# lucidrains/audiolm-pytorch

Hardware: NVIDIA H100
Metric: CoarseTransformer tokens/sec fwd+bwd seq2048 (higher is better)
Workload: dtype bf16

## Files before the change

audiolm_pytorch_b200/csrc/attn_fwd_wgmma.cu:

```cuda
#include "alm_common.cuh"
#include "ptx_sm90.cuh"

namespace alm {

constexpr int ATT_BM = 128;
constexpr int ATT_BN = 128;
constexpr int ATT_THREADS = 384;
template <int D>
struct AttFwdCfg {
  static constexpr int KV_STAGES = D == 128 ? 3 : 4;
  static constexpr int HALF_BYTES = 128 * SwizzledTile<D>::ROW_BYTES;
  static constexpr int TILE_BYTES = 128 * D * 2;
  static constexpr int SMEM_BYTES = TILE_BYTES * (1 + 2 * KV_STAGES) + 256;
};

struct AttnFwdParams {
  __nv_bfloat16* o;
  float* lse;
  const uint32_t* kmask;
  int kb_stride;
  const float* bias;
  long long bias_hs, bias_rs;
  long long ldo, lse_stride;
  int b, h, n_q, n_k;
  int causal;
  float scale_log2;
  int n_q_pad;
  uint32_t drop_row0;
  DropoutArgs drop;
};

__device__ __forceinline__ float att_ex2(float x) {
  float y;
  asm("ex2.approx.ftz.f32 %0, %1;" : "=f"(y) : "f"(x));
  return y;
}

__device__ __forceinline__ uint64_t attn_fwd_keep_bits(const DropoutArgs& d, uint32_t qrow, uint32_t kbase, int c_lane) {
  const uint32_t odd = qrow & 1u;
  uint64_t bits = 0;
#pragma unroll
  for (int kk = 0; kk < ATT_BN / 16; ++kk) {
    const uint32_t j0 = kbase + 16 * kk + c_lane;
    const uint4 own = dropout_draw(d, qrow, j0 + odd);
    const uint32_t ra = __shfl_xor_sync(0xffffffffu, odd ? own.x : own.y, 4);
    const uint32_t rb = __shfl_xor_sync(0xffffffffu, odd ? own.z : own.w, 4);
    const uint4 other = odd ? make_uint4(0u, ra, 0u, rb) : make_uint4(ra, 0u, rb, 0u);
#pragma unroll
    for (int c = 0; c < 2; ++c) {
      const uint4 dr = (uint32_t)c == odd ? own : other;
#pragma unroll
      for (int half = 0; half < 2; ++half)
#pragma unroll
        for (int h = 0; h < 2; ++h)
          if (dropout_pick(d, dr, qrow + 8 * h, j0 + 8 * half + c)) bits |= 1ull << (8 * kk + 4 * half + 2 * h + c);
    }
  }
  return bits;
}

template <int ATT_D, bool HAS_BIAS, bool DROPOUT>
__global__ void __launch_bounds__(ATT_THREADS, 1)
mqa_attn_fwd_kernel(const __grid_constant__ CUtensorMap tmQ, const __grid_constant__ CUtensorMap tmK,
                    const __grid_constant__ CUtensorMap tmV, const AttnFwdParams p) {
  using Tile = SwizzledTile<ATT_D>;
  using Cfg = AttFwdCfg<ATT_D>;
  constexpr int ATT_KV_STAGES = Cfg::KV_STAGES, ATT_TILE_BYTES = Cfg::TILE_BYTES, HALF = Cfg::HALF_BYTES;
  constexpr bool REG_HANDOFF = ATT_D == 128;
  extern __shared__ __align__(1024) uint8_t smem_raw[];
  uint8_t* smem = smem_raw;
  if ((smem_u32(smem) & 1023u) != 0) __trap();
  uint8_t* sQ = smem;
  uint8_t* sK = sQ + ATT_TILE_BYTES;
  uint8_t* sV = sK + ATT_KV_STAGES * ATT_TILE_BYTES;
  uint64_t* bars = reinterpret_cast<uint64_t*>(sV + ATT_KV_STAGES * ATT_TILE_BYTES);
  uint64_t* q_full = bars;
  uint64_t* kv_full = bars + 1;
  uint64_t* kv_empty = kv_full + ATT_KV_STAGES;

  const int warp = threadIdx.x >> 5;
  const int lane = threadIdx.x & 31;
  const int wg = warp >> 2;
  const int n_qblocks = (p.n_q + ATT_BM - 1) / ATT_BM;
  const int qb = n_qblocks - 1 - (int)blockIdx.x;
  const int head = blockIdx.y;
  const int batch = blockIdx.z;
  const int q0 = qb * ATT_BM;
  const int off = p.n_k - p.n_q;
  int kv_end = p.n_k;
  if (p.causal) kv_end = min(p.n_k, q0 + ATT_BM + off);
  const int n_tiles = kv_end > 0 ? (kv_end + ATT_BN - 1) / ATT_BN : 0;

  if (threadIdx.x == 0) {
    tma_prefetch_desc(&tmQ);
    tma_prefetch_desc(&tmK);
    tma_prefetch_desc(&tmV);
    mbar_init(q_full, 1);
    for (int i = 0; i < ATT_KV_STAGES; ++i) {
      mbar_init(&kv_full[i], 1);
      mbar_init(&kv_empty[i], 8);
    }
    fence_mbar_init();
  }
  __syncthreads();

  if (wg == 0) {
    if constexpr (REG_HANDOFF) setmaxnreg_dec<40>();
    if (warp == 0 && n_tiles > 0) {
      if (elect_one_sync()) {
        mbar_arrive_expect_tx(q_full, ATT_TILE_BYTES);
#pragma unroll
        for (int hf = 0; hf < Tile::HALVES; ++hf)
          tma_load_3d(sQ + hf * HALF, &tmQ, q_full, head * ATT_D + hf * Tile::HW, q0, batch);
      }
      __syncwarp();
      int stage = 0;
      uint32_t phase = 0;
      for (int j = 0; j < n_tiles; ++j) {
        mbar_wait(&kv_empty[stage], phase ^ 1u);
        if (elect_one_sync()) {
          mbar_arrive_expect_tx(&kv_full[stage], 2 * ATT_TILE_BYTES);
#pragma unroll
          for (int hf = 0; hf < Tile::HALVES; ++hf) {
            tma_load_3d(sK + stage * ATT_TILE_BYTES + hf * HALF, &tmK, &kv_full[stage], hf * Tile::HW, j * ATT_BN, batch);
            tma_load_3d(sV + stage * ATT_TILE_BYTES + hf * HALF, &tmV, &kv_full[stage], hf * Tile::HW, j * ATT_BN, batch);
          }
        }
        __syncwarp();
        if (++stage == ATT_KV_STAGES) { stage = 0; phase ^= 1u; }
      }
    }
    return;
  }

  if constexpr (REG_HANDOFF) setmaxnreg_inc<232>();
  const int cw = wg - 1;
  const int r_base = cw * 64 + (warp & 3) * 16 + (lane >> 2);
  const int c_lane = 2 * (lane & 3);
  constexpr float kLog2e = 1.4426950408889634f;
  float m_run[2] = {-INFINITY, -INFINITY}, l_run[2] = {0.f, 0.f};
  float o_acc[ATT_D / 2];
#pragma unroll
  for (int d = 0; d < ATT_D / 2; ++d) o_acc[d] = 0.f;
  int q_limit[2];
  [[maybe_unused]] const float* brow[2];
#pragma unroll
  for (int h = 0; h < 2; ++h) {
    const int qi = q0 + r_base + 8 * h;
    q_limit[h] = min(p.causal ? qi + off : p.n_k - 1, p.n_k - 1);
    if constexpr (HAS_BIAS) brow[h] = p.bias + (long long)head * p.bias_hs + (long long)min(qi, p.n_q - 1) * p.bias_rs;
  }
  const uint32_t* mrow = p.kmask ? p.kmask + (long long)batch * p.kb_stride : nullptr;
  const uint32_t q_addr = smem_u32(sQ) + cw * 64 * Tile::ROW_BYTES;
  [[maybe_unused]] const uint32_t drop_row =
      p.drop_row0 + ((uint32_t)batch * p.h + head) * (uint32_t)p.n_q_pad + q0 + r_base;

  if (n_tiles > 0) mbar_wait(q_full, 0);
  int stage = 0;
  uint32_t phase = 0;
  for (int j = 0; j < n_tiles; ++j) {
    mbar_wait(&kv_full[stage], phase);
    const uint32_t k_addr = smem_u32(sK + stage * ATT_TILE_BYTES);
    const uint32_t v_addr = smem_u32(sV + stage * ATT_TILE_BYTES);
    float s[ATT_BN / 2];
    wgmma_fence();
#pragma unroll
    for (int k = 0; k < ATT_D / 16; ++k)
      wgmma_ss<ATT_BN>(s, Tile::kmajor(q_addr, k, HALF), Tile::kmajor(k_addr, k, HALF), k > 0 ? 1u : 0u);
    wgmma_commit();
    [[maybe_unused]] uint64_t keep = 0;
    if constexpr (DROPOUT) keep = attn_fwd_keep_bits(p.drop, drop_row, j * ATT_BN, c_lane);
    wgmma_wait<0>();
    wgmma_fence_acc(s);

    const int kbase = j * ATT_BN;
    const bool tile_full = mrow == nullptr && kbase + ATT_BN <= p.n_k && (!p.causal || kbase + ATT_BN - 1 <= q0 + off);
    uint32_t valid[4] = {0xFFFFFFFFu, 0xFFFFFFFFu, 0xFFFFFFFFu, 0xFFFFFFFFu};
    if (!tile_full && mrow != nullptr) {
      const uint4 mv = __ldg(reinterpret_cast<const uint4*>(mrow + j * 4));
      valid[0] = mv.x; valid[1] = mv.y; valid[2] = mv.z; valid[3] = mv.w;
    }
    uint32_t pa[ATT_BN / 16][4];
#pragma unroll
    for (int h = 0; h < 2; ++h) {
#pragma unroll
      for (int g = 0; g < ATT_BN / 8; ++g)
#pragma unroll
        for (int c = 0; c < 2; ++c) {
          const int col = 8 * g + c_lane + c;
          float v = s[4 * g + 2 * h + c] * p.scale_log2;
          if constexpr (HAS_BIAS) {
            if (kbase + col < p.bias_rs) v = fmaf(__ldg(brow[h] + kbase + col), kLog2e, v);
          }
          if (!tile_full) {
            const bool ok = kbase + col <= q_limit[h] && ((valid[col >> 5] >> (col & 31)) & 1u);
            if (!ok) v = -INFINITY;
          }
          s[4 * g + 2 * h + c] = v;
        }
      float m_tile = -INFINITY;
#pragma unroll
      for (int g = 0; g < ATT_BN / 8; ++g) m_tile = fmaxf(m_tile, fmaxf(s[4 * g + 2 * h], s[4 * g + 2 * h + 1]));
      m_tile = fmaxf(m_tile, __shfl_xor_sync(0xffffffffu, m_tile, 1));
      m_tile = fmaxf(m_tile, __shfl_xor_sync(0xffffffffu, m_tile, 2));
      const float m_new = fmaxf(m_run[h], m_tile);
      const float m_use = (m_new == -INFINITY) ? 0.f : m_new;
      const float alpha = att_ex2(m_run[h] - m_use);
      float l_tile = 0.f;
#pragma unroll
      for (int g = 0; g < ATT_BN / 8; ++g)
#pragma unroll
        for (int c = 0; c < 2; ++c) {
          const float pv = att_ex2(s[4 * g + 2 * h + c] - m_use);
          s[4 * g + 2 * h + c] = pv;
          l_tile += pv;
        }
      l_run[h] = fmaf(l_run[h], alpha, l_tile);
      m_run[h] = m_new;
#pragma unroll
      for (int g = 0; g < ATT_D / 8; ++g) {
        o_acc[4 * g + 2 * h] *= alpha;
        o_acc[4 * g + 2 * h + 1] *= alpha;
      }
    }
    if constexpr (DROPOUT) {
#pragma unroll
      for (int e = 0; e < ATT_BN / 2; ++e) s[e] = ((keep >> e) & 1u) ? s[e] * p.drop.scale : 0.f;
    }
#pragma unroll
    for (int kk = 0; kk < ATT_BN / 16; ++kk) {
      pa[kk][0] = pack_bf16x2(s[8 * kk + 0], s[8 * kk + 1]);
      pa[kk][1] = pack_bf16x2(s[8 * kk + 2], s[8 * kk + 3]);
      pa[kk][2] = pack_bf16x2(s[8 * kk + 4], s[8 * kk + 5]);
      pa[kk][3] = pack_bf16x2(s[8 * kk + 6], s[8 * kk + 7]);
    }
    wgmma_fence_acc(o_acc);
    wgmma_fence();
#pragma unroll
    for (int kk = 0; kk < ATT_BN / 16; ++kk)
      wgmma_rs<ATT_D, 1>(o_acc, pa[kk], Tile::mnmajor(v_addr, kk, HALF), 1u);
    wgmma_commit();
    wgmma_wait<0>();
    wgmma_fence_acc(o_acc);
    if (lane == 0) mbar_arrive(&kv_empty[stage]);
    if (++stage == ATT_KV_STAGES) { stage = 0; phase ^= 1u; }
  }

#pragma unroll
  for (int h = 0; h < 2; ++h) {
    float l_tot = l_run[h];
    l_tot += __shfl_xor_sync(0xffffffffu, l_tot, 1);
    l_tot += __shfl_xor_sync(0xffffffffu, l_tot, 2);
    const int qi = q0 + r_base + 8 * h;
    if (qi < p.n_q) {
      const float inv = l_tot > 0.f ? 1.f / l_tot : 0.f;
      __nv_bfloat16* dst = p.o + ((long long)batch * p.n_q + qi) * p.ldo + head * ATT_D + c_lane;
#pragma unroll
      for (int g = 0; g < ATT_D / 8; ++g)
        *reinterpret_cast<uint32_t*>(dst + 8 * g) = pack_bf16x2(o_acc[4 * g + 2 * h] * inv, o_acc[4 * g + 2 * h + 1] * inv);
      if (p.lse != nullptr && (lane & 3) == 0) {
        const float lse = l_tot > 0.f ? (m_run[h] + log2f(l_tot)) : INFINITY;
        p.lse[((long long)batch * p.h + head) * p.lse_stride + qi] = lse;
      }
    }
  }
}

}

namespace alm {
__global__ void pack_key_mask_kernel(const uint8_t* __restrict__ mask, uint32_t* __restrict__ bits, int n_k, int words,
                                     long long total) {
  const long long i = (long long)blockIdx.x * (blockDim.x >> 5) + (threadIdx.x >> 5);
  if (i >= total) return;
  const long long b = i / words;
  const int k = (int)(i - b * words) * 32 + (threadIdx.x & 31);
  const bool on = k < n_k && mask[b * n_k + k] != 0;
  const uint32_t v = __ballot_sync(0xffffffffu, on);
  if ((threadIdx.x & 31) == 0) bits[i] = v;
}
}

extern "C" int alm_pack_key_mask(const void* key_mask, void* bits, int b, int n_k, alm_stream_t stream_) {
  using namespace alm;
  cudaStream_t stream = reinterpret_cast<cudaStream_t>(stream_);
  ALM_REQUIRE(key_mask && bits && b > 0 && n_k > 0, ALM_ERR_ARG);
  const int words = (n_k + 127) / 128 * 4;
  const long long total = (long long)b * words;
  const long long blocks = ceil_div(total, 8LL);
  ALM_REQUIRE(blocks <= INT_MAX, ALM_ERR_UNSUPPORTED);
  pack_key_mask_kernel<<<(unsigned)blocks, 256, 0, stream>>>(reinterpret_cast<const uint8_t*>(key_mask),
                                                            reinterpret_cast<uint32_t*>(bits), n_k, words, total);
  ALM_CHECK_LAUNCH();
  ALM_LAUNCHED(1);
  return ALM_OK;
}

namespace alm {
template <int D>
static int attn_fwd_launch(const void* q, int64_t ldq, const void* k, int64_t ldk, int64_t k_bstride, const void* v,
                           int64_t ldv, int64_t v_bstride, const void* key_mask, void* o, int64_t ldo, float* lse,
                           const float* bias, int b, bool drop, AttnFwdParams p, cudaStream_t stream) {
  using Tile = SwizzledTile<D>;
  constexpr int SMEM = AttFwdCfg<D>::SMEM_BYTES;
  const int h = p.h, n_q = p.n_q, n_k = p.n_k;
  static bool attr_set = false;
  if (!attr_set) {
    ALM_CUDA_OK(cudaFuncSetAttribute(mqa_attn_fwd_kernel<D, false, false>, cudaFuncAttributeMaxDynamicSharedMemorySize, SMEM));
    ALM_CUDA_OK(cudaFuncSetAttribute(mqa_attn_fwd_kernel<D, true, false>, cudaFuncAttributeMaxDynamicSharedMemorySize, SMEM));
    ALM_CUDA_OK(cudaFuncSetAttribute(mqa_attn_fwd_kernel<D, false, true>, cudaFuncAttributeMaxDynamicSharedMemorySize, SMEM));
    ALM_CUDA_OK(cudaFuncSetAttribute(mqa_attn_fwd_kernel<D, true, true>, cudaFuncAttributeMaxDynamicSharedMemorySize, SMEM));
    attr_set = true;
  }
  constexpr int kMaxGridZ = 65535;
  const int n_launch = ceil_div(b, kMaxGridZ);
  for (int b0 = 0; b0 < b; b0 += kMaxGridZ) {
    const int nb = min(b - b0, kMaxGridZ);
    CUtensorMap tmQ, tmK, tmV;
    {
      uint64_t dims[3] = {(uint64_t)h * D, (uint64_t)n_q, (uint64_t)nb};
      uint64_t strides[3] = {2, (uint64_t)ldq * 2, (uint64_t)n_q * ldq * 2};
      uint32_t box[3] = {Tile::HW, ATT_BM, 1};
      int rc = make_tensor_map(&tmQ, reinterpret_cast<const __nv_bfloat16*>(q) + (long long)b0 * n_q * ldq, 2, 3, dims,
                               strides, box, Tile::SWIZZLE);
      if (rc != ALM_OK) return rc;
    }
    {
      uint64_t dims[3] = {(uint64_t)D, (uint64_t)n_k, (uint64_t)nb};
      uint64_t strides[3] = {2, (uint64_t)ldk * 2, (uint64_t)k_bstride * 2};
      uint32_t box[3] = {Tile::HW, ATT_BN, 1};
      int rc = make_tensor_map(&tmK, reinterpret_cast<const __nv_bfloat16*>(k) + (long long)b0 * k_bstride, 2, 3, dims,
                               strides, box, Tile::SWIZZLE);
      if (rc != ALM_OK) return rc;
      strides[1] = (uint64_t)ldv * 2;
      strides[2] = (uint64_t)v_bstride * 2;
      rc = make_tensor_map(&tmV, reinterpret_cast<const __nv_bfloat16*>(v) + (long long)b0 * v_bstride, 2, 3, dims,
                           strides, box, Tile::SWIZZLE);
      if (rc != ALM_OK) return rc;
    }
    p.o = reinterpret_cast<__nv_bfloat16*>(o) + (long long)b0 * n_q * ldo;
    p.lse = lse != nullptr ? lse + (long long)b0 * h * p.lse_stride : nullptr;
    p.kmask = key_mask != nullptr ? reinterpret_cast<const uint32_t*>(key_mask) + (long long)b0 * p.kb_stride : nullptr;
    p.b = nb;
    p.drop_row0 = (uint32_t)((long long)b0 * h * p.n_q_pad);
    const dim3 grid((n_q + ATT_BM - 1) / ATT_BM, h, nb);
    if (bias != nullptr && drop)
      mqa_attn_fwd_kernel<D, true, true><<<grid, ATT_THREADS, SMEM, stream>>>(tmQ, tmK, tmV, p);
    else if (bias != nullptr)
      mqa_attn_fwd_kernel<D, true, false><<<grid, ATT_THREADS, SMEM, stream>>>(tmQ, tmK, tmV, p);
    else if (drop)
      mqa_attn_fwd_kernel<D, false, true><<<grid, ATT_THREADS, SMEM, stream>>>(tmQ, tmK, tmV, p);
    else
      mqa_attn_fwd_kernel<D, false, false><<<grid, ATT_THREADS, SMEM, stream>>>(tmQ, tmK, tmV, p);
    ALM_CHECK_LAUNCH();
  }
  ALM_LAUNCHED(n_launch);
  return ALM_OK;
}
}

extern "C" int alm_mqa_attn_fwd_dh(const void* q, int64_t ldq, const void* k, int64_t ldk, int64_t k_bstride,
                                   const void* v, int64_t ldv, int64_t v_bstride, const void* key_mask, void* o,
                                   int64_t ldo, float* lse, int64_t lse_stride, const float* bias,
                                   int64_t bias_hstride, int64_t bias_rstride, int b, int h, int n_q, int n_k,
                                   int causal, float scale, float dropout_p, uint64_t seed, uint32_t site,
                                   int dim_head, alm_stream_t stream_) {
  using namespace alm;
  cudaStream_t stream = reinterpret_cast<cudaStream_t>(stream_);
  ALM_REQUIRE(dim_head == 32 || dim_head == 64 || dim_head == 128, ALM_ERR_UNSUPPORTED);
  ALM_REQUIRE(q && k && v && o, ALM_ERR_ARG);
  ALM_REQUIRE(b > 0 && h > 0 && n_q > 0 && n_k > 0 && n_k >= n_q, ALM_ERR_ARG);
  ALM_REQUIRE(dropout_p >= 0.f && dropout_p < 1.f, ALM_ERR_ARG);
  ALM_REQUIRE((long long)b * h * ((n_q + 127) / 128 * 128) < (1ll << 32), ALM_ERR_UNSUPPORTED);
  ALM_REQUIRE(ldq % 8 == 0 && ldk % 8 == 0 && ldv % 8 == 0 && ldo % 8 == 0, ALM_ERR_ALIGN);
  ALM_REQUIRE(k_bstride % 8 == 0 && v_bstride % 8 == 0, ALM_ERR_ALIGN);
  ALM_REQUIRE((reinterpret_cast<uintptr_t>(o) & 15u) == 0, ALM_ERR_ALIGN);
  if (bias != nullptr) {
    ALM_REQUIRE(bias_rstride >= n_k && bias_rstride % 4 == 0 && bias_hstride % 4 == 0, ALM_ERR_ALIGN);
    ALM_REQUIRE((reinterpret_cast<uintptr_t>(bias) & 15u) == 0, ALM_ERR_ALIGN);
  }

  AttnFwdParams p;
  p.kb_stride = (n_k + 127) / 128 * 4;
  p.bias = bias;
  p.bias_hs = bias_hstride;
  p.bias_rs = bias_rstride;
  p.ldo = ldo;
  p.lse_stride = lse_stride;
  p.h = h; p.n_q = n_q; p.n_k = n_k;
  p.causal = causal;
  p.scale_log2 = scale * 1.4426950408889634f;
  p.n_q_pad = (n_q + 127) / 128 * 128;
  p.drop = make_dropout_args(dropout_p, seed, site);
  const bool drop = dropout_p > 0.f;
#define ALM_ATT_FWD(DD) \
  attn_fwd_launch<DD>(q, ldq, k, ldk, k_bstride, v, ldv, v_bstride, key_mask, o, ldo, lse, bias, b, drop, p, stream)
  if (dim_head == 32) return ALM_ATT_FWD(32);
  if (dim_head == 64) return ALM_ATT_FWD(64);
  return ALM_ATT_FWD(128);
#undef ALM_ATT_FWD
}

extern "C" int alm_mqa_attn_fwd(const void* q, int64_t ldq, const void* k, int64_t ldk, int64_t k_bstride,
                                const void* v, int64_t ldv, int64_t v_bstride, const void* key_mask, void* o,
                                int64_t ldo, float* lse, int64_t lse_stride, const float* bias, int64_t bias_hstride,
                                int64_t bias_rstride, int b, int h, int n_q, int n_k, int causal, float scale,
                                float dropout_p, uint64_t seed, uint32_t site, alm_stream_t stream_) {
  return alm_mqa_attn_fwd_dh(q, ldq, k, ldk, k_bstride, v, ldv, v_bstride, key_mask, o, ldo, lse, lse_stride, bias,
                             bias_hstride, bias_rstride, b, h, n_q, n_k, causal, scale, dropout_p, seed, site, 64,
                             stream_);
}
```

include/alm_b200.h:

```cpp
#ifndef ALM_B200_H_
#define ALM_B200_H_

#include <stddef.h>
#include <stdint.h>

#ifdef __cplusplus
extern "C" {
#endif

typedef struct CUstream_st* alm_stream_t;

typedef enum alm_status {
  ALM_OK = 0,
  ALM_ERR_ARG = -1,
  ALM_ERR_ALIGN = -2,
  ALM_ERR_CUDA = -3,
  ALM_ERR_UNSUPPORTED = -4
} alm_status;

int alm_version(void);
const char* alm_status_string(int code);
unsigned long long alm_launch_count(void);
void alm_reset_launch_count(void);

int alm_gemm_bf16(const void* A, int a_mn, int64_t lda, int64_t strideA, const void* B, int b_mn, int64_t ldb,
                  int64_t strideB, void* C, int c_fp32, int64_t ldc, int64_t strideC, int M, int N, int K, int batch,
                  float alpha, const float* bias, int acc_mode, int split_k, alm_stream_t stream);

int alm_embed_gather(const float* const* tables, int n_tables, const int32_t* src, float* out, int M, int d,
                     alm_stream_t stream);
int alm_embed_scatter(float* const* grad_tables, int n_tables, const int32_t* src, const float* dout, int M, int d,
                      alm_stream_t stream);
int alm_pack_key_mask(const void* key_mask, void* bits, int b, int n_k, alm_stream_t stream);
int alm_mqa_attn_fwd(const void* q, int64_t ldq, const void* k, int64_t ldk, int64_t k_bstride, const void* v,
                     int64_t ldv, int64_t v_bstride, const void* key_mask, void* o, int64_t ldo, float* lse,
                     int64_t lse_stride, const float* bias, int64_t bias_hstride, int64_t bias_rstride, int b, int h,
                     int n_q, int n_k, int causal, float scale, float dropout_p, uint64_t seed, uint32_t site,
                     alm_stream_t stream);

int alm_mqa_attn_fwd_dh(const void* q, int64_t ldq, const void* k, int64_t ldk, int64_t k_bstride, const void* v,
                        int64_t ldv, int64_t v_bstride, const void* key_mask, void* o, int64_t ldo, float* lse,
                        int64_t lse_stride, const float* bias, int64_t bias_hstride, int64_t bias_rstride, int b,
                        int h, int n_q, int n_k, int causal, float scale, float dropout_p, uint64_t seed,
                        uint32_t site, int dim_head, alm_stream_t stream);

int alm_mqa_attn_bwd(const void* q, int64_t ldq, const void* k, int64_t ldk, int64_t k_bstride, const void* v,
                     int64_t ldv, int64_t v_bstride, const void* d_o, int64_t lddo, const void* key_mask,
                     const float* lse, const float* delta, int n_q_pad, void* dq, int64_t lddq, float* dq_acc,
                     void* dk, int64_t lddk, void* dv, int64_t lddv, const float* bias, float* dbias,
                     int64_t bias_hstride, int64_t bias_rstride, int b, int h, int n_q, int n_k, int causal,
                     float scale, float dropout_p, uint64_t seed, uint32_t site, alm_stream_t stream);
int alm_attn_delta(const void* o, int64_t ldo, const void* d_o, int64_t lddo, float* delta ,
                   int64_t delta_stride, float* dq_acc, int b, int h, int n, alm_stream_t stream);

int alm_mqa_attn_bwd_dh(const void* q, int64_t ldq, const void* k, int64_t ldk, int64_t k_bstride, const void* v,
                        int64_t ldv, int64_t v_bstride, const void* d_o, int64_t lddo, const void* key_mask,
                        const float* lse, const float* delta, int n_q_pad, void* dq, int64_t lddq, float* dq_acc,
                        void* dk, int64_t lddk, void* dv, int64_t lddv, const float* bias, float* dbias,
                        int64_t bias_hstride, int64_t bias_rstride, int b, int h, int n_q, int n_k, int causal,
                        float scale, float dropout_p, uint64_t seed, uint32_t site, int dim_head, alm_stream_t stream);
int alm_attn_delta_dh(const void* o, int64_t ldo, const void* d_o, int64_t lddo, float* delta ,
                      int64_t delta_stride, float* dq_acc, int b, int h, int n, int dim_head, alm_stream_t stream);

int alm_bias_gather_fwd(const float* table, const int32_t* idx, const float* override_h, float* out, int heads,
                        int n_q, int n_k, int64_t ld, alm_stream_t stream);
int alm_bias_gather_bwd(const float* dbias, const int32_t* idx, float* dtable, float* doverride, int heads, int n_q,
                        int n_k, int64_t ld, alm_stream_t stream);

int alm_gemv_bf16(const void* x, int64_t ldx, const void* W, int64_t ldw, void* out, int c_fp32, int64_t ldo,
                  const float* bias, int rows, int N, int K, alm_stream_t stream);
int alm_kv_append(const void* kv_new, int64_t ld, void* k_cache, void* v_cache, int64_t cache_bstride,
                  const int32_t* len, int max_len, int b, alm_stream_t stream);
int alm_mqa_attn_decode(const void* q, int64_t ldq, const void* k_cache, const void* v_cache, int64_t cache_bstride,
                        const int32_t* len, int max_len, const void* key_mask, int64_t mask_bstride, const float* bias,
                        int64_t bias_ld, void* o, int64_t ldo,
                        float* workspace , int splits, int b, int h,
                        float scale, alm_stream_t stream);
int alm_kv_append_dh(const void* kv_new, int64_t ld, void* k_cache, void* v_cache, int64_t cache_bstride,
                     const int32_t* len, int max_len, int b, int dim_head, alm_stream_t stream);
int alm_mqa_attn_decode_dh(const void* q, int64_t ldq, const void* k_cache, const void* v_cache, int64_t cache_bstride,
                           const int32_t* len, int max_len, const void* key_mask, int64_t mask_bstride,
                           const float* bias, int64_t bias_ld, void* o, int64_t ldo, float* workspace, int splits,
                           int b, int h, float scale, int dim_head, alm_stream_t stream);
int alm_decode_bias_row(const float* table, int rows, const float* override_h, const int32_t* u, const int32_t* cls,
                        int c, const int32_t* len, int max_len, float* out, int64_t ld, int h, alm_stream_t stream);

int alm_gemm_head_ce_tiles(int V);
int alm_gemm_head_ce(const void* X, int64_t ldx, const void* W, int64_t ldw, const float* bias, const int64_t* labels,
                     int64_t ignore_index, int mode, float* part, float* lab_logit, const float* lse,
                     const float* scale_num, const float* scale_den, void* dlogits, int64_t ldd, int M, int V, int K,
                     alm_stream_t stream);
int alm_ce_finish(const float* part, int tiles, const float* lab_logit, const int64_t* labels, int64_t ignore_index,
                  float* lse, float* loss_rows, int M, alm_stream_t stream);

int alm_decode_stack_grid(void);
int alm_decode_stack_plan(int b, int d, int heads, int inner, int n_layers, int32_t* staged);
int alm_decode_stack_plan_dh(int b, int d, int heads, int inner, int n_layers, int dim_head, int32_t* staged);
int64_t alm_decode_stack_scratch_bytes(int b, int d, int heads, int inner);
int64_t alm_decode_stack_trace_offset(int b, int d, int heads, int inner);
int alm_decode_stack_step(const void* layer_table, int n_layers, const float* x, void* out, const float* final_gamma,
                          int32_t* len, int max_len, int64_t cache_bstride, const void* key_mask, int64_t mask_bstride,
                          void* scratch, int64_t scratch_bytes, int b, int d, int heads, int inner, int value_residual,
                          float scale, int grid_ctas , alm_stream_t stream);

int alm_hc_pre_fwd(const void* R_in, const void* Y, const float* beta_prev, const float* x_expand,
                   const float* gamma_hc, const float* dyn_alpha, const float* dyn_beta, const float* static_alpha,
                   const float* static_beta, const float* alpha_scale, const float* beta_scale,
                   const float* ln_gamma, void* R_out, void* bin, void* xn, float* beta_out, float* aux, int M,
                   int d, int streams, alm_stream_t stream);
int alm_hc_pre_bwd(const void* R_in, const void* Y, const float* beta_prev, const float* x_expand,
                   const float* gamma_hc, const float* dyn_alpha, const float* dyn_beta, const float* static_alpha,
                   const float* static_beta, const float* alpha_scale, const float* beta_scale,
                   const float* ln_gamma, const float* aux, const void* dR_out, const void* dxn,
                   const void* dbin_extra, const float* dbeta, void* dR_in, void* dY, float* dbeta_prev,
                   float* dx_expand, float dx_scale, float* g_gamma_hc, float* g_dyn_alpha, float* g_dyn_beta,
                   float* g_static_alpha, float* g_static_beta, float* g_alpha_scale, float* g_beta_scale,
                   float* g_ln_gamma, int M, int d, int streams, alm_stream_t stream);
int alm_hc_post_fwd(const void* R_in, const void* Y, const float* beta_prev, const float* ln_gamma, void* out,
                    float* stats, int M, int d, int streams, alm_stream_t stream);
int alm_hc_post_bwd(const void* R_in, const void* Y, const float* beta_prev, const float* ln_gamma,
                    const float* stats, const void* dout, void* dR_in, void* dY, float* dbeta_prev,
                    float* g_ln_gamma, int M, int d, int streams, alm_stream_t stream);

int alm_resid_ln_fwd(const float* r, const void* y, const float* gamma, float* r_new, void* xn, void* rb, float* stats,
                     int M, int d, alm_stream_t stream);
int alm_resid_ln_bwd(const float* r_new, const float* gamma, const float* stats, const float* dr_out, const void* dxn,
                     const void* dextra, float* dr, void* dr_bf16, float* g_gamma, float out_scale, int M, int d,
                     alm_stream_t stream);

int alm_geglu_ln_fwd(const void* h, int64_t ldh, int gate_off, const float* gamma, void* gn, int64_t ldg,
                     float* stats, int M, int inner, int inner_pad, float dropout_p, uint64_t seed, uint32_t site,
                     alm_stream_t stream);
int alm_geglu_ln_bwd(const void* h, int64_t ldh, int gate_off, const float* gamma, const float* stats,
                     const void* dgn, int64_t ldg, void* dh, float* g_gamma, int M, int inner, int inner_pad,
                     float dropout_p, uint64_t seed, uint32_t site, alm_stream_t stream);

int alm_dropout_bf16(void* x, int64_t ld, int64_t M, int C, float p, uint64_t seed, uint32_t site,
                     alm_stream_t stream);

int alm_ce_fwd_bwd(const float* logits, int64_t ldl, const int64_t* labels, int64_t ignore_index, float* loss_rows,
                   void* dlogits, int64_t ldd, const float* scale_num, const float* scale_den, int rows, int V,
                   int Vpad, alm_stream_t stream);

int alm_topk_gumbel_sample(const float* logits, int64_t ldl, const float* uniform, int64_t ldu, int64_t* ids, int rows,
                           int V, int k, float temperature, alm_stream_t stream);

int alm_axpby_bf16(const void* x, int64_t ldx, float alpha, const void* y, int64_t ldy, float beta, void* out,
                   int64_t ldout, int64_t rows, int cols, alm_stream_t stream);
int alm_cast_pad_bf16(const float* src, int64_t lds, void* dst, int64_t ldd, int64_t rows, int cols, int cols_pad,
                      alm_stream_t stream);
int alm_cast_pad_multi(const int64_t* desc_dev, int n, alm_stream_t stream);
int alm_scale_by_scalar_bf16(void* x, const float* s, int64_t n, alm_stream_t stream);

int alm_causal_conv1d_fwd(const float* x, const float* w, const float* bias, const float* residual, float* y, int B,
                          int Cin, int Cout, int T, int K, int stride, int dilation, int pad_mode, int act_elu,
                          int w_packed, alm_stream_t stream);
int alm_residual_unit_fwd(const float* x, const float* w7_packed, const float* b7, const float* w1_packed,
                          const float* b1, float* y, int B, int C, int T, int dilation, int pad_mode,
                          alm_stream_t stream);
int alm_codec_se_fp32(const float* y, const float* x, const float* w1_folded, const float* b1, const float* w2,
                      const float* b2, float* out, int B, int C, int Ci, int T, alm_stream_t stream);
int alm_codec_first_conv(const float* x, const float* w, const float* bias, void* y, int B, int T, int Cout, int K,
                         int pad_mode, alm_stream_t stream);
int alm_codec_ru_tc(const void* x, void* y, const void* w_units, const float* b7, const float* b1, int B, int C, int T,
                    int dilation, int pad_mode, int out_phases, alm_stream_t stream);
int alm_codec_conv_tc(const void* x, void* y, const void* w_units, const float* bias, int B, int Cin, int Cout, int Tin,
                      int K, int stride, int pad_mode, int out_phases, int out_fp32, int upsample, alm_stream_t stream);
int alm_codec_ru_se_tc(const void* x, void* y, const void* w_units, const float* b7, const float* b1, const float* se_b1,
                       const float* se_b2, int B, int C, int se_ci, int T, int dilation, int pad_mode, int out_phases,
                       alm_stream_t stream);
int alm_codec_pack_c8s(const float* x, void* y, int B, int n, int C, alm_stream_t stream);
int alm_codec_last_conv(const void* x, const float* w, const float* bias, float* y, int B, int T, int Cin, int K,
                        int pad_mode, alm_stream_t stream);
long long alm_codec_gate_loop_workspace(int B, int C, int T, int tc);
int alm_codec_gate_loop_fp32(const float* x, const float* proj, float* y, float* workspace, int B, int C, int T,
                             alm_stream_t stream);
int alm_codec_gate_loop_tc(const void* x, const void* w_units, void* y, float* workspace, int B, int C, int T,
                           alm_stream_t stream);
int alm_causal_convT1d_fwd(const float* x, const float* w, const float* bias, float* y, int B, int Cin, int Cout,
                           int n, int stride, alm_stream_t stream);
int alm_rvq_encode(const float* x, int64_t ldx, const float* codebooks, float* e2_workspace, float* quantized,
                   int64_t ldq, int64_t* indices, int64_t ldi, int N, int D, int C, int Q, alm_stream_t stream);
int alm_rvq_pack_codebooks(const float* codebooks, void* packed, float* e2, int64_t rows, int D, alm_stream_t stream);
int alm_rvq_prepare(const float* x, int64_t ldx, float* r, float* quantized, int64_t ldq, void* rp, int N, int D,
                    alm_stream_t stream);
int alm_rvq_select(const float* scores, int64_t lds, const float* e2, const float* codebook, float* r, float* quantized,
                   int64_t ldq, void* rp, int64_t* indices, int64_t ldi, int N, int D, int C, int write_rp,
                   alm_stream_t stream);

int alm_rvq_decode(const int64_t* indices, int64_t ldi, const float* codebooks, float* out, int64_t ldo, int N, int D,
                   int C, int Q, alm_stream_t stream);

int alm_sq_encode(const float* x, int64_t ldx, int N, int groups, int Dg, int mode, const float* w_in, const float* b_in,
                  const float* w_out_t, const float* b_out, const float* consts, const int32_t* ints, int dc, int Q,
                  float* quantized, int64_t ldq, void* indices, int idx64, alm_stream_t stream);
int alm_sq_decode(const void* indices, int idx64, int Qi, int N, int groups, int Dg, int mode, const float* w_out_t,
                  const float* b_out, const float* consts, const int32_t* ints, int dc, int Q, float* out, int64_t ldo,
                  alm_stream_t stream);

#ifdef __cplusplus
}
#endif
#endif
```

Measured before the change: 747,800.

## Pipeline QK^T of next tile with PV of current tile in D=64 attention forward

Adds a pipelined variant of the MQA attention forward kernel for head dim 64 without bias or dropout. It issues the next tile's S=QK^T wgmma before the current tile's PV wgmma and computes softmax while PV runs, so tensor-core work overlaps the exp/max math. It also switches that path to register handoff and simplifies mask evaluation with precomputed shifted bit words. The old serial path stays available through a flag, and optional clock64 trace stamps are added. The cost is more live registers (two S tiles plus O), which risks spills, and more complex barrier phase handling.

New measurement: 756,100 (median of 6 runs). 1.01x the previous value.

```diff
diff --git a/audiolm_pytorch_b200/csrc/attn_fwd_wgmma.cu b/audiolm_pytorch_b200/csrc/attn_fwd_wgmma.cu
--- a/audiolm_pytorch_b200/csrc/attn_fwd_wgmma.cu
+++ b/audiolm_pytorch_b200/csrc/attn_fwd_wgmma.cu
@@ -59,14 +59,91 @@
   return bits;
 }
 
-template <int ATT_D, bool HAS_BIAS, bool DROPOUT>
+__device__ __forceinline__ bool attn_fwd_tile_keys(const AttnFwdParams& p, const uint32_t* mrow, int j, int q0, int off,
+                                                   uint32_t (&valid)[4]) {
+  const int kbase = j * ATT_BN;
+  const bool tile_full = mrow == nullptr && kbase + ATT_BN <= p.n_k && (!p.causal || kbase + ATT_BN - 1 <= q0 + off);
+  valid[0] = valid[1] = valid[2] = valid[3] = 0xFFFFFFFFu;
+  if (!tile_full && mrow != nullptr) {
+    const uint4 mv = __ldg(reinterpret_cast<const uint4*>(mrow + j * 4));
+    valid[0] = mv.x; valid[1] = mv.y; valid[2] = mv.z; valid[3] = mv.w;
+  }
+  return tile_full;
+}
+
+__device__ __forceinline__ float attn_fwd_softmax_row(float (&s)[ATT_BN / 2], int h, int kbase, bool tile_full,
+                                                      const uint32_t (&valid)[4], int q_limit, const AttnFwdParams& p,
+                                                      int c_lane, float& m_run, float& l_run) {
+#pragma unroll
+  for (int g = 0; g < ATT_BN / 8; ++g)
+#pragma unroll
+    for (int c = 0; c < 2; ++c) s[4 * g + 2 * h + c] *= p.scale_log2;
+  if (!tile_full) {
+    const int lim = q_limit - kbase - c_lane;
+    uint32_t w[4];
+#pragma unroll
+    for (int i = 0; i < 4; ++i) w[i] = valid[i] >> c_lane;
+#pragma unroll
+    for (int g = 0; g < ATT_BN / 8; ++g)
+#pragma unroll
+      for (int c = 0; c < 2; ++c) {
+        const bool ok = 8 * g + c <= lim && ((w[g >> 2] >> (8 * (g & 3) + c)) & 1u);
+        if (!ok) s[4 * g + 2 * h + c] = -INFINITY;
+      }
+  }
+  float m_tile = -INFINITY;
+#pragma unroll
+  for (int g = 0; g < ATT_BN / 8; ++g) m_tile = fmaxf(m_tile, fmaxf(s[4 * g + 2 * h], s[4 * g + 2 * h + 1]));
+  m_tile = fmaxf(m_tile, __shfl_xor_sync(0xffffffffu, m_tile, 1));
+  m_tile = fmaxf(m_tile, __shfl_xor_sync(0xffffffffu, m_tile, 2));
+  const float m_new = fmaxf(m_run, m_tile);
+  const float m_use = (m_new == -INFINITY) ? 0.f : m_new;
+  const float alpha = att_ex2(m_run - m_use);
+  float l_tile = 0.f;
+#pragma unroll
+  for (int g = 0; g < ATT_BN / 8; ++g)
+#pragma unroll
+    for (int c = 0; c < 2; ++c) {
+      const float pv = att_ex2(s[4 * g + 2 * h + c] - m_use);
+      s[4 * g + 2 * h + c] = pv;
+      l_tile += pv;
+    }
+  l_run = fmaf(l_run, alpha, l_tile);
+  m_run = m_new;
+  return alpha;
+}
+
+__device__ __forceinline__ void attn_fwd_pack_p(const float (&s)[ATT_BN / 2], uint32_t (&pa)[ATT_BN / 16][4]) {
+#pragma unroll
+  for (int kk = 0; kk < ATT_BN / 16; ++kk) {
+    pa[kk][0] = pack_bf16x2(s[8 * kk + 0], s[8 * kk + 1]);
+    pa[kk][1] = pack_bf16x2(s[8 * kk + 2], s[8 * kk + 3]);
+    pa[kk][2] = pack_bf16x2(s[8 * kk + 4], s[8 * kk + 5]);
+    pa[kk][3] = pack_bf16x2(s[8 * kk + 6], s[8 * kk + 7]);
+  }
+}
+
+#ifdef ALM_ATTN_FWD_TRACE
+constexpr int AF_TRACE_TILES = 32, AF_TRACE_STAMPS = 8;
+__device__ long long g_attn_fwd_trace[2][AF_TRACE_TILES][AF_TRACE_STAMPS];
+#define AF_STAMP(t, i)                                                                                 \
+  do {                                                                                                 \
+    if (blockIdx.x == 0 && blockIdx.y == 0 && blockIdx.z == 0 && (threadIdx.x & 127) == 0 &&          \
+        (t) < AF_TRACE_TILES)                                                                          \
+      g_attn_fwd_trace[(threadIdx.x >> 7) - 1][(t)][i] = clock64();                                    \
+  } while (0)
+#else
+#define AF_STAMP(t, i)
+#endif
+
+template <int ATT_D, bool HAS_BIAS, bool DROPOUT, bool PIPE = false>
 __global__ void __launch_bounds__(ATT_THREADS, 1)
 mqa_attn_fwd_kernel(const __grid_constant__ CUtensorMap tmQ, const __grid_constant__ CUtensorMap tmK,
                     const __grid_constant__ CUtensorMap tmV, const AttnFwdParams p) {
   using Tile = SwizzledTile<ATT_D>;
   using Cfg = AttFwdCfg<ATT_D>;
   constexpr int ATT_KV_STAGES = Cfg::KV_STAGES, ATT_TILE_BYTES = Cfg::TILE_BYTES, HALF = Cfg::HALF_BYTES;
-  constexpr bool REG_HANDOFF = ATT_D == 128;
+  constexpr bool REG_HANDOFF = ATT_D == 128 || PIPE;
   extern __shared__ __align__(1024) uint8_t smem_raw[];
   uint8_t* smem = smem_raw;
   if ((smem_u32(smem) & 1023u) != 0) __trap();
@@ -158,92 +235,182 @@
   if (n_tiles > 0) mbar_wait(q_full, 0);
   int stage = 0;
   uint32_t phase = 0;
-  for (int j = 0; j < n_tiles; ++j) {
-    mbar_wait(&kv_full[stage], phase);
-    const uint32_t k_addr = smem_u32(sK + stage * ATT_TILE_BYTES);
-    const uint32_t v_addr = smem_u32(sV + stage * ATT_TILE_BYTES);
-    float s[ATT_BN / 2];
-    wgmma_fence();
-#pragma unroll
-    for (int k = 0; k < ATT_D / 16; ++k)
-      wgmma_ss<ATT_BN>(s, Tile::kmajor(q_addr, k, HALF), Tile::kmajor(k_addr, k, HALF), k > 0 ? 1u : 0u);
-    wgmma_commit();
-    [[maybe_unused]] uint64_t keep = 0;
-    if constexpr (DROPOUT) keep = attn_fwd_keep_bits(p.drop, drop_row, j * ATT_BN, c_lane);
-    wgmma_wait<0>();
-    wgmma_fence_acc(s);
-
-    const int kbase = j * ATT_BN;
-    const bool tile_full = mrow == nullptr && kbase + ATT_BN <= p.n_k && (!p.causal || kbase + ATT_BN - 1 <= q0 + off);
-    uint32_t valid[4] = {0xFFFFFFFFu, 0xFFFFFFFFu, 0xFFFFFFFFu, 0xFFFFFFFFu};
-    if (!tile_full && mrow != nullptr) {
-      const uint4 mv = __ldg(reinterpret_cast<const uint4*>(mrow + j * 4));
-      valid[0] = mv.x; valid[1] = mv.y; valid[2] = mv.z; valid[3] = mv.w;
-    }
+  if constexpr (PIPE) {
+    static_assert(!HAS_BIAS && !DROPOUT, "the pipelined schedule is built without bias and dropout");
+    auto issue_s = [&](float (&s)[ATT_BN / 2], int st) {
+      const uint32_t k_addr = smem_u32(sK + st * ATT_TILE_BYTES);
+      wgmma_fence();
+#pragma unroll
+      for (int k = 0; k < ATT_D / 16; ++k)
+        wgmma_ss<ATT_BN>(s, Tile::kmajor(q_addr, k, HALF), Tile::kmajor(k_addr, k, HALF), k > 0 ? 1u : 0u);
+      wgmma_commit();
+    };
+    auto softmax = [&](float (&s)[ATT_BN / 2], int j, float (&alpha)[2]) {
+      uint32_t valid[4];
+      const bool tile_full = attn_fwd_tile_keys(p, mrow, j, q0, off, valid);
+#pragma unroll
+      for (int h = 0; h < 2; ++h)
+        alpha[h] = attn_fwd_softmax_row(s, h, j * ATT_BN, tile_full, valid, q_limit[h], p, c_lane, m_run[h], l_run[h]);
+    };
+    auto rescale_o = [&](const float (&alpha)[2]) {
+#pragma unroll
+      for (int h = 0; h < 2; ++h)
+#pragma unroll
+        for (int g = 0; g < ATT_D / 8; ++g) {
+          o_acc[4 * g + 2 * h] *= alpha[h];
+          o_acc[4 * g + 2 * h + 1] *= alpha[h];
+        }
+    };
     uint32_t pa[ATT_BN / 16][4];
-#pragma unroll
-    for (int h = 0; h < 2; ++h) {
-#pragma unroll
-      for (int g = 0; g < ATT_BN / 8; ++g)
-#pragma unroll
-        for (int c = 0; c < 2; ++c) {
-          const int col = 8 * g + c_lane + c;
-          float v = s[4 * g + 2 * h + c] * p.scale_log2;
-          if constexpr (HAS_BIAS) {
-            if (kbase + col < p.bias_rs) v = fmaf(__ldg(brow[h] + kbase + col), kLog2e, v);
+    float s[ATT_BN / 2], alpha[2];
+    if (n_tiles > 0) {
+      AF_STAMP(0, 0);
+      mbar_wait(&kv_full[0], 0);
+      AF_STAMP(0, 1);
+      issue_s(s, 0);
+      AF_STAMP(0, 2);
+      wgmma_wait<0>();
+      wgmma_fence_acc(s);
+      AF_STAMP(0, 3);
+      softmax(s, 0, alpha);
+      rescale_o(alpha);
+      attn_fwd_pack_p(s, pa);
+      AF_STAMP(0, 4);
+    }
+    auto issue_pv = [&]() {
+      const uint32_t v_addr = smem_u32(sV + stage * ATT_TILE_BYTES);
+      wgmma_fence_acc(o_acc);
+      wgmma_fence();
+#pragma unroll
+      for (int kk = 0; kk < ATT_BN / 16; ++kk)
+        wgmma_rs<ATT_D, 1>(o_acc, pa[kk], Tile::mnmajor(v_addr, kk, HALF), 1u);
+      wgmma_commit();
+    };
+    for (int j = 0; j + 1 < n_tiles; ++j) {
+      const int nstage = stage + 1 == ATT_KV_STAGES ? 0 : stage + 1;
+      AF_STAMP(j + 1, 0);
+      mbar_wait(&kv_full[nstage], nstage == 0 ? phase ^ 1u : phase);
+      AF_STAMP(j + 1, 1);
+      issue_s(s, nstage);
+      AF_STAMP(j + 1, 2);
+      issue_pv();
+      AF_STAMP(j, 5);
+      wgmma_wait<1>();
+      wgmma_fence_acc(s);
+      AF_STAMP(j + 1, 3);
+      softmax(s, j + 1, alpha);
+      AF_STAMP(j + 1, 4);
+      wgmma_wait<0>();
+      wgmma_fence_acc(o_acc);
+      AF_STAMP(j, 6);
+      if (lane == 0) mbar_arrive(&kv_empty[stage]);
+      rescale_o(alpha);
+      attn_fwd_pack_p(s, pa);
+      stage = nstage;
+      if (stage == 0) phase ^= 1u;
+    }
+    if (n_tiles > 0) {
+      issue_pv();
+      AF_STAMP(n_tiles - 1, 5);
+      wgmma_wait<0>();
+      wgmma_fence_acc(o_acc);
+      AF_STAMP(n_tiles - 1, 6);
+    }
+  } else {
+    for (int j = 0; j < n_tiles; ++j) {
+      AF_STAMP(j, 0);
+      mbar_wait(&kv_full[stage], phase);
+      AF_STAMP(j, 1);
+      const uint32_t k_addr = smem_u32(sK + stage * ATT_TILE_BYTES);
+      const uint32_t v_addr = smem_u32(sV + stage * ATT_TILE_BYTES);
+      float s[ATT_BN / 2];
+      wgmma_fence();
+#pragma unroll
+      for (int k = 0; k < ATT_D / 16; ++k)
+        wgmma_ss<ATT_BN>(s, Tile::kmajor(q_addr, k, HALF), Tile::kmajor(k_addr, k, HALF), k > 0 ? 1u : 0u);
+      wgmma_commit();
+      AF_STAMP(j, 2);
+      [[maybe_unused]] uint64_t keep = 0;
+      if constexpr (DROPOUT) keep = attn_fwd_keep_bits(p.drop, drop_row, j * ATT_BN, c_lane);
+      wgmma_wait<0>();
+      wgmma_fence_acc(s);
+      AF_STAMP(j, 3);
+
+      const int kbase = j * ATT_BN;
+      const bool tile_full = mrow == nullptr && kbase + ATT_BN <= p.n_k && (!p.causal || kbase + ATT_BN - 1 <= q0 + off);
+      uint32_t valid[4] = {0xFFFFFFFFu, 0xFFFFFFFFu, 0xFFFFFFFFu, 0xFFFFFFFFu};
+      if (!tile_full && mrow != nullptr) {
+        const uint4 mv = __ldg(reinterpret_cast<const uint4*>(mrow + j * 4));
+        valid[0] = mv.x; valid[1] = mv.y; valid[2] = mv.z; valid[3] = mv.w;
+      }
+      uint32_t pa[ATT_BN / 16][4];
+#pragma unroll
+      for (int h = 0; h < 2; ++h) {
+#pragma unroll
+        for (int g = 0; g < ATT_BN / 8; ++g)
+#pragma unroll
+          for (int c = 0; c < 2; ++c) {
+            const int col = 8 * g + c_lane + c;
+            float v = s[4 * g + 2 * h + c] * p.scale_log2;
+            if constexpr (HAS_BIAS) {
+              if (kbase + col < p.bias_rs) v = fmaf(__ldg(brow[h] + kbase + col), kLog2e, v);
+            }
+            if (!tile_full) {
+              const bool ok = kbase + col <= q_limit[h] && ((valid[col >> 5] >> (col & 31)) & 1u);
+              if (!ok) v = -INFINITY;
+            }
+            s[4 * g + 2 * h + c] = v;
           }
-          if (!tile_full) {
-            const bool ok = kbase + col <= q_limit[h] && ((valid[col >> 5] >> (col & 31)) & 1u);
-            if (!ok) v = -INFINITY;
+        float m_tile = -INFINITY;
+#pragma unroll
+        for (int g = 0; g < ATT_BN / 8; ++g) m_tile = fmaxf(m_tile, fmaxf(s[4 * g + 2 * h], s[4 * g + 2 * h + 1]));
+        m_tile = fmaxf(m_tile, __shfl_xor_sync(0xffffffffu, m_tile, 1));
+        m_tile = fmaxf(m_tile, __shfl_xor_sync(0xffffffffu, m_tile, 2));
+        const float m_new = fmaxf(m_run[h], m_tile);
+        const float m_use = (m_new == -INFINITY) ? 0.f : m_new;
+        const float alpha = att_ex2(m_run[h] - m_use);
+        float l_tile = 0.f;
+#pragma unroll
+        for (int g = 0; g < ATT_BN / 8; ++g)
+#pragma unroll
+          for (int c = 0; c < 2; ++c) {
+            const float pv = att_ex2(s[4 * g + 2 * h + c] - m_use);
+            s[4 * g + 2 * h + c] = pv;
+            l_tile += pv;
           }
-          s[4 * g + 2 * h + c] = v;
+        l_run[h] = fmaf(l_run[h], alpha, l_tile);
+        m_run[h] = m_new;
+#pragma unroll
+        for (int g = 0; g < ATT_D / 8; ++g) {
+          o_acc[4 * g + 2 * h] *= alpha;
+          o_acc[4 * g + 2 * h + 1] *= alpha;
         }
-      float m_tile = -INFINITY;
-#pragma unroll
-      for (int g = 0; g < ATT_BN / 8; ++g) m_tile = fmaxf(m_tile, fmaxf(s[4 * g + 2 * h], s[4 * g + 2 * h + 1]));
-      m_tile = fmaxf(m_tile, __shfl_xor_sync(0xffffffffu, m_tile, 1));
-      m_tile = fmaxf(m_tile, __shfl_xor_sync(0xffffffffu, m_tile, 2));
-      const float m_new = fmaxf(m_run[h], m_tile);
-      const float m_use = (m_new == -INFINITY) ? 0.f : m_new;
-      const float alpha = att_ex2(m_run[h] - m_use);
-      float l_tile = 0.f;
-#pragma unroll
-      for (int g = 0; g < ATT_BN / 8; ++g)
-#pragma unroll
-        for (int c = 0; c < 2; ++c) {
-          const float pv = att_ex2(s[4 * g + 2 * h + c] - m_use);
-          s[4 * g + 2 * h + c] = pv;
-          l_tile += pv;
-        }
-      l_run[h] = fmaf(l_run[h], alpha, l_tile);
-      m_run[h] = m_new;
-#pragma unroll
-      for (int g = 0; g < ATT_D / 8; ++g) {
-        o_acc[4 * g + 2 * h] *= alpha;
-        o_acc[4 * g + 2 * h + 1] *= alpha;
-      }
-    }
-    if constexpr (DROPOUT) {
-#pragma unroll
-      for (int e = 0; e < ATT_BN / 2; ++e) s[e] = ((keep >> e) & 1u) ? s[e] * p.drop.scale : 0.f;
-    }
-#pragma unroll
-    for (int kk = 0; kk < ATT_BN / 16; ++kk) {
-      pa[kk][0] = pack_bf16x2(s[8 * kk + 0], s[8 * kk + 1]);
-      pa[kk][1] = pack_bf16x2(s[8 * kk + 2], s[8 * kk + 3]);
-      pa[kk][2] = pack_bf16x2(s[8 * kk + 4], s[8 * kk + 5]);
-      pa[kk][3] = pack_bf16x2(s[8 * kk + 6], s[8 * kk + 7]);
-    }
-    wgmma_fence_acc(o_acc);
-    wgmma_fence();
-#pragma unroll
-    for (int kk = 0; kk < ATT_BN / 16; ++kk)
-      wgmma_rs<ATT_D, 1>(o_acc, pa[kk], Tile::mnmajor(v_addr, kk, HALF), 1u);
-    wgmma_commit();
-    wgmma_wait<0>();
-    wgmma_fence_acc(o_acc);
-    if (lane == 0) mbar_arrive(&kv_empty[stage]);
-    if (++stage == ATT_KV_STAGES) { stage = 0; phase ^= 1u; }
+      }
+      if constexpr (DROPOUT) {
+#pragma unroll
+        for (int e = 0; e < ATT_BN / 2; ++e) s[e] = ((keep >> e) & 1u) ? s[e] * p.drop.scale : 0.f;
+      }
+#pragma unroll
+      for (int kk = 0; kk < ATT_BN / 16; ++kk) {
+        pa[kk][0] = pack_bf16x2(s[8 * kk + 0], s[8 * kk + 1]);
+        pa[kk][1] = pack_bf16x2(s[8 * kk + 2], s[8 * kk + 3]);
+        pa[kk][2] = pack_bf16x2(s[8 * kk + 4], s[8 * kk + 5]);
+        pa[kk][3] = pack_bf16x2(s[8 * kk + 6], s[8 * kk + 7]);
+      }
+      AF_STAMP(j, 4);
+      wgmma_fence_acc(o_acc);
+      wgmma_fence();
+#pragma unroll
+      for (int kk = 0; kk < ATT_BN / 16; ++kk)
+        wgmma_rs<ATT_D, 1>(o_acc, pa[kk], Tile::mnmajor(v_addr, kk, HALF), 1u);
+      wgmma_commit();
+      AF_STAMP(j, 5);
+      wgmma_wait<0>();
+      wgmma_fence_acc(o_acc);
+      AF_STAMP(j, 6);
+      if (lane == 0) mbar_arrive(&kv_empty[stage]);
+      if (++stage == ATT_KV_STAGES) { stage = 0; phase ^= 1u; }
+    }
   }
 
 #pragma unroll
@@ -300,7 +467,7 @@
 template <int D>
 static int attn_fwd_launch(const void* q, int64_t ldq, const void* k, int64_t ldk, int64_t k_bstride, const void* v,
                            int64_t ldv, int64_t v_bstride, const void* key_mask, void* o, int64_t ldo, float* lse,
-                           const float* bias, int b, bool drop, AttnFwdParams p, cudaStream_t stream) {
+                           const float* bias, int b, bool drop, bool serial, AttnFwdParams p, cudaStream_t stream) {
   using Tile = SwizzledTile<D>;
   constexpr int SMEM = AttFwdCfg<D>::SMEM_BYTES;
   const int h = p.h, n_q = p.n_q, n_k = p.n_k;
@@ -310,6 +477,9 @@
     ALM_CUDA_OK(cudaFuncSetAttribute(mqa_attn_fwd_kernel<D, true, false>, cudaFuncAttributeMaxDynamicSharedMemorySize, SMEM));
     ALM_CUDA_OK(cudaFuncSetAttribute(mqa_attn_fwd_kernel<D, false, true>, cudaFuncAttributeMaxDynamicSharedMemorySize, SMEM));
     ALM_CUDA_OK(cudaFuncSetAttribute(mqa_attn_fwd_kernel<D, true, true>, cudaFuncAttributeMaxDynamicSharedMemorySize, SMEM));
+    if constexpr (D == 64)
+      ALM_CUDA_OK(cudaFuncSetAttribute(mqa_attn_fwd_kernel<64, false, false, true>,
+                                       cudaFuncAttributeMaxDynamicSharedMemorySize, SMEM));
     attr_set = true;
   }
   constexpr int kMaxGridZ = 65535;
@@ -350,6 +520,8 @@
       mqa_attn_fwd_kernel<D, true, false><<<grid, ATT_THREADS, SMEM, stream>>>(tmQ, tmK, tmV, p);
     else if (drop)
       mqa_attn_fwd_kernel<D, false, true><<<grid, ATT_THREADS, SMEM, stream>>>(tmQ, tmK, tmV, p);
+    else if (D == 64 && !serial)
+      mqa_attn_fwd_kernel<D, false, false, D == 64><<<grid, ATT_THREADS, SMEM, stream>>>(tmQ, tmK, tmV, p);
     else
       mqa_attn_fwd_kernel<D, false, false><<<grid, ATT_THREADS, SMEM, stream>>>(tmQ, tmK, tmV, p);
     ALM_CHECK_LAUNCH();
@@ -367,6 +539,8 @@
                                    int dim_head, alm_stream_t stream_) {
   using namespace alm;
   cudaStream_t stream = reinterpret_cast<cudaStream_t>(stream_);
+  const bool serial = (dim_head & ALM_ATTN_SERIAL) != 0;
+  dim_head &= ~ALM_ATTN_SERIAL;
   ALM_REQUIRE(dim_head == 32 || dim_head == 64 || dim_head == 128, ALM_ERR_UNSUPPORTED);
   ALM_REQUIRE(q && k && v && o, ALM_ERR_ARG);
   ALM_REQUIRE(b > 0 && h > 0 && n_q > 0 && n_k > 0 && n_k >= n_q, ALM_ERR_ARG);
@@ -394,12 +568,20 @@
   p.drop = make_dropout_args(dropout_p, seed, site);
   const bool drop = dropout_p > 0.f;
 #define ALM_ATT_FWD(DD) \
-  attn_fwd_launch<DD>(q, ldq, k, ldk, k_bstride, v, ldv, v_bstride, key_mask, o, ldo, lse, bias, b, drop, p, stream)
+  attn_fwd_launch<DD>(q, ldq, k, ldk, k_bstride, v, ldv, v_bstride, key_mask, o, ldo, lse, bias, b, drop, serial, p, \
+                      stream)
   if (dim_head == 32) return ALM_ATT_FWD(32);
   if (dim_head == 64) return ALM_ATT_FWD(64);
   return ALM_ATT_FWD(128);
 #undef ALM_ATT_FWD
 }
+
+#ifdef ALM_ATTN_FWD_TRACE
+extern "C" int alm_attn_fwd_trace_read(long long* dst) {
+  ALM_CUDA_OK(cudaMemcpyFromSymbol(dst, alm::g_attn_fwd_trace, sizeof(alm::g_attn_fwd_trace)));
+  return ALM_OK;
+}
+#endif
 
 extern "C" int alm_mqa_attn_fwd(const void* q, int64_t ldq, const void* k, int64_t ldk, int64_t k_bstride,
                                 const void* v, int64_t ldv, int64_t v_bstride, const void* key_mask, void* o,
diff --git a/include/alm_b200.h b/include/alm_b200.h
--- a/include/alm_b200.h
+++ b/include/alm_b200.h
@@ -38,6 +38,7 @@
                      int n_q, int n_k, int causal, float scale, float dropout_p, uint64_t seed, uint32_t site,
                      alm_stream_t stream);
 
+#define ALM_ATTN_SERIAL 0x100
 int alm_mqa_attn_fwd_dh(const void* q, int64_t ldq, const void* k, int64_t ldk, int64_t k_bstride, const void* v,
                         int64_t ldv, int64_t v_bstride, const void* key_mask, void* o, int64_t ldo, float* lse,
                         int64_t lse_stride, const float* bias, int64_t bias_hstride, int64_t bias_rstride, int b,
```
